# henryhungle/MTN

Measured on AMD Instinct MI355X. Metric: train-step samples/sec (d_model=512, 6L MTN), higher is better.
Workload: dtype bf16; 1 GPU; cfg2: d_model=512 N=6 h=8 d_ff=2048 |V|=3000 Q/H/C/T=20/128/40/20 frames=[32, 32] ft=[2048, 128]; batch_per_gpu=32, global_batch=32, parallelism=dp1, hip_graph=True, rccl_ranks=1

## Files before the change

mtn_amd/build.py:

```python
import os
import shutil
import subprocess
import sys
from concurrent.futures import ThreadPoolExecutor

HERE = os.path.dirname(os.path.abspath(__file__))
CSRC = os.path.join(HERE, "csrc")
OBJ = os.path.join(HERE, "build")
LIB = os.path.join(HERE, "libmtn_hip.so")
SOURCES = ["gemm.hip", "layernorm.hip", "attention.hip", "fused.hip", "fused_bwd.hip", "elementwise.hip", "sublayer.hip", "losshead.hip", "assemble.hip", "select.hip", "diverse.hip", "sample.hip", "score.hip", "constrain.hip", "ensemble.hip", "mbr.hip", "eval.hip", "scst.hip", "average.hip", "gradnorm.hip", "gradaccum.hip", "gemm_k512.hip", "decode.hip"]
FLAGS = ["--offload-arch=gfx950", "-O3", "-std=c++17", "-fPIC"]
SAFE_LIB = os.path.join(HERE, "libmtn_hip_safewaits.so")
SAFE_SOURCES = ["fused.hip", "fused_bwd.hip"]


def _headers_mtime() -> float:
    hs = [os.path.join(CSRC, f) for f in os.listdir(CSRC) if f.endswith(".h")] + [os.path.join(HERE, "..", "include", "mtn_hip.h")]
    return max(os.path.getmtime(h) for h in hs if os.path.exists(h))


def _stale() -> bool:
    if not os.path.exists(LIB):
        return True
    t = os.path.getmtime(LIB)
    deps = [os.path.join(CSRC, f) for f in os.listdir(CSRC)] + [os.path.join(HERE, "..", "include", "mtn_hip.h")]
    return any(os.path.getmtime(d) > t for d in deps if os.path.exists(d))


def build(force: bool = False, verbose: bool = True) -> str:
    if not force and not _stale():
        return LIB
    hipcc = shutil.which("hipcc") or "/opt/rocm/bin/hipcc"
    if not os.path.exists(hipcc):
        raise RuntimeError("hipcc not found: cannot build libmtn_hip.so")
    os.makedirs(OBJ, exist_ok=True)
    ht = _headers_mtime()
    todo = []
    for s in SOURCES:
        src, obj = os.path.join(CSRC, s), os.path.join(OBJ, s[:-4] + ".o")
        if force or not os.path.exists(obj) or os.path.getmtime(obj) < max(os.path.getmtime(src), ht):
            todo.append((src, obj))

    def cc(job):
        cmd = [hipcc] + FLAGS + ["-c", job[0], "-o", job[1]]
        if verbose:
            print(" ".join(cmd), flush=True)
        subprocess.check_call(cmd)

    with ThreadPoolExecutor(max(1, min(len(todo), os.cpu_count() or 1))) as ex:
        list(ex.map(cc, todo))
    cmd = [hipcc, "--offload-arch=gfx950", "-shared", "-fPIC", "-o", LIB + ".tmp"] + [os.path.join(OBJ, s[:-4] + ".o") for s in SOURCES]
    if verbose:
        print(" ".join(cmd), flush=True)
    subprocess.check_call(cmd)
    os.replace(LIB + ".tmp", LIB)
    return LIB


def build_safe_waits(verbose: bool = True) -> str:
    build(verbose=verbose)
    srcs = [os.path.join(CSRC, s) for s in SAFE_SOURCES]
    if os.path.exists(SAFE_LIB) and os.path.getmtime(SAFE_LIB) >= max(os.path.getmtime(LIB), max(os.path.getmtime(s) for s in srcs)):
        return SAFE_LIB
    hipcc = shutil.which("hipcc") or "/opt/rocm/bin/hipcc"

    def cc(s):
        obj = os.path.join(OBJ, s[:-4] + "_safewaits.o")
        cmd = [hipcc] + FLAGS + ["-DMTN_SAFE_WAITS", "-c", os.path.join(CSRC, s), "-o", obj]
        if verbose:
            print(" ".join(cmd), flush=True)
        subprocess.check_call(cmd)
        return obj

    with ThreadPoolExecutor(len(SAFE_SOURCES)) as ex:
        safe = list(ex.map(cc, SAFE_SOURCES))
    objs = safe + [os.path.join(OBJ, s[:-4] + ".o") for s in SOURCES if s not in SAFE_SOURCES]
    subprocess.check_call([hipcc, "--offload-arch=gfx950", "-shared", "-fPIC", "-o", SAFE_LIB + ".tmp"] + objs)
    os.replace(SAFE_LIB + ".tmp", SAFE_LIB)
    return SAFE_LIB


if __name__ == "__main__":
    build(force="--force" in sys.argv)
    print(LIB)
    print(build_safe_waits())
```

mtn_amd/csrc/common.h:

```cpp
#pragma once
#include <hip/hip_runtime.h>
#include <stdint.h>
#include <stdio.h>
#include <string.h>

#include "../../include/mtn_hip.h"

typedef unsigned short bf16_t;
typedef __attribute__((ext_vector_type(8))) __bf16 bf16x8_t;
typedef __attribute__((ext_vector_type(4))) float f32x4_t;

void mtn_set_error(const char* fmt, ...);
#define MTN_CHECK_ARG(cond, msg)                         \
    do {                                                 \
        if (!(cond)) {                                   \
            mtn_set_error("%s: %s", __func__, msg);      \
            return MTN_ERR_ARG;                          \
        }                                                \
    } while (0)
#define MTN_CHECK_LAUNCH()                                                        \
    do {                                                                          \
        hipError_t e__ = hipGetLastError();                                       \
        if (e__ != hipSuccess) {                                                  \
            mtn_set_error("%s: launch failed: %s", __func__, hipGetErrorString(e__)); \
            return MTN_ERR_LAUNCH;                                                \
        }                                                                         \
    } while (0)

struct MtnEnvVar { const char* name; int gen; bool set; char val[56]; };
const char* mtn_env_lookup(MtnEnvVar* v);
#define MTN_ENV(NAME) ([]() -> const char* { static MtnEnvVar v_ = {NAME, -1, false, {0}}; return mtn_env_lookup(&v_); }())

__device__ __forceinline__ float bf16_to_f32(bf16_t b) { return __uint_as_float(((uint32_t)b) << 16); }
__device__ __forceinline__ bf16_t f32_to_bf16(float f) {
    uint32_t u = __float_as_uint(f);
    if ((u & 0x7fffffffu) > 0x7f800000u) return (bf16_t)((u >> 16) | 0x40);
    u += 0x7fffu + ((u >> 16) & 1u);
    return (bf16_t)(u >> 16);
}

template <typename T> struct LP;
template <> struct LP<float> {
    static constexpr int EPV = 4;
    static constexpr int KSTEP = 16;
    __device__ static __forceinline__ float to_f32(float v) { return v; }
    __device__ static __forceinline__ float from_f32(float v) { return v; }
};
template <> struct LP<bf16_t> {
    static constexpr int EPV = 8;
    static constexpr int KSTEP = 32;
    __device__ static __forceinline__ float to_f32(bf16_t v) { return bf16_to_f32(v); }
    __device__ static __forceinline__ bf16_t from_f32(float v) { return f32_to_bf16(v); }
};

typedef __attribute__((ext_vector_type(4))) unsigned u32x4_t;
// ... 147 lines not shown
```

mtn_amd/csrc/fused.hip:

```cpp
#include "fused_common.h"
#include "gemm_k512_tile.h"

struct FhMember {
    int kind;
    int rows;
    int rows_per_wg;
    int nslice;
    int a, m, blk;
    int mt;
    int hg, sg;
    int late_v;
    int nks;
    int ncols;
    int ld_out;
    float eps;
    const float* x;
    const float* ln_a;
    const float* ln_b;
    const bf16_t* w;
    const float* bias;
    const bf16_t* mem;
    bf16_t* xn;
    float* mean;
    float* rstd;
    bf16_t* out;
    bf16_t* kv;
    const uint8_t* mask;
    long mask_sb, mask_sq;
    mtn_dropout drop;
    bf16_t* o;
    float* lse;
    int b_off;
};
struct FhGroup {
    int count;
    int stop;
#ifdef FH_TIMELINE
    unsigned long long* dbg;
#endif
    int wg_start[FH_MAX_MEMBERS + 1];
    FhMember m[FH_MAX_MEMBERS];
    int rider_base;
    GkRider kv;
};
static_assert(sizeof(FhGroup) <= 4096, "FhGroup travels by value in the kernel arguments");

struct FhLds { int gains, xn, xm, qi, ki, vi, mask, total; };
__host__ __device__ inline FhLds fh_lds_map(int mt, bool raw, int key_rows, int pad_rows, int mask_bytes, int ffn_blocks = 0, bool late_v = false) {
    FhLds L;
    L.gains = 0;
    L.xn = 4096 + 1024;
    const int krows = ((key_rows + pad_rows + 7) & ~7);
    if (late_v) {
        L.vi = L.xn;
        const int top = mt * 16 * FH_ROWB > krows * FH_HROWB ? mt * 16 * FH_ROWB : krows * FH_HROWB;
        L.xm = L.xn + top;
        L.qi = L.xm;
        L.ki = L.qi + mt * 16 * FH_HROWB;
        L.mask = L.ki + krows * FH_HROWB;
        L.total = L.mask + ((mask_bytes + 15) & ~15);
        return L;
    }
    L.xm = L.xn + mt * 16 * FH_ROWB;
    L.qi = L.xm + (raw ? mt * 16 * FH_ROWB : 0);
    L.ki = L.qi + mt * 16 * (ffn_blocks ? ffn_blocks * FH_HROWB : FH_HROWB);
    L.vi = L.ki + krows * FH_HROWB;
    L.mask = L.vi + krows * FH_HROWB;
    L.total = L.mask + ((mask_bytes + 15) & ~15);
// ... 474 lines not shown
        }
        __syncthreads();
        if (live && kr == 0) {
            for (int k = 1; k < nks; ++k) {
                const float* pk = (const float*)ki_s + (size_t)(pair * (nks - 1) + k - 1) * (FH_PART_FLOATS * 64) + lane;
                const float mo = pk[16 * 64], lo = pk[17 * 64];
                const float mn = fmaxf(mrun, mo);
                const float wa = (mrun == -INFINITY) ? 0.f : __expf(mrun - mn), wb = (mo == -INFINITY) ? 0.f : __expf(mo - mn);
                lrun = lrun * wa + lo * wb;
                mrun = mn;
#pragma unroll
                for (int nt = 0; nt < 4; ++nt)
#pragma unroll
                    for (int r = 0; r < 4; ++r) ot[nt][r] = ot[nt][r] * wa + pk[(nt * 4 + r) * 64] * wb;
            }
            finish(si, qt, ot, mrun, lrun);
        }
    }
    FH_STAMP(9);
    FH_STAMP_CLK(11);
}

template <int NP>
__global__ __launch_bounds__(FH_THREADS) void fused_head_fwd_kernel(const FhGroup G) {
    extern __shared__ __attribute__((aligned(16))) unsigned char smem[];
    FH_STAMP(0);
    FH_STAMP_CLK(10);
    if ((int)blockIdx.x >= G.wg_start[FH_MAX_MEMBERS]) {
        const int r = (int)blockIdx.x - G.rider_base;
        if (r >= 0 && r < G.kv.units) gk_rider_unit(G.kv, r, smem);
        return;
    }
    int g = 0;
    while (g + 1 < G.count && (int)blockIdx.x >= G.wg_start[g + 1]) ++g;
    const FhMember& M = G.m[g];
    const int t = (int)blockIdx.x - G.wg_start[g];
    const int xcd = t & 7, j = t >> 3;
    const int hpg = M.nslice / M.hg;
    const int slice = (xcd % M.hg) * hpg + (j % hpg), rb = (j / hpg) * M.sg + (xcd / M.hg);
    FH_STAMP(12);
    if (rb * M.rows_per_wg >= M.rows) return;
    if constexpr (NP == 4) {
        if (M.mt <= 2) fh_body<NP, 2>(G, M, slice, rb, smem);
        else fh_body<NP, 4>(G, M, slice, rb, smem);
    } else {
        if (M.mt <= 2) fh_body<NP, 2>(G, M, slice, rb, smem);
        else if (M.mt == 3) fh_body<NP, 3>(G, M, slice, rb, smem);
        else if (M.mt == 4) fh_body<NP, 4>(G, M, slice, rb, smem);
        else fh_body<NP, 5>(G, M, slice, rb, smem);
    }
}

static int fh_enabled = -1;
extern "C" int mtn_fused_enable(int on) {
    const int prev = fh_enabled;
    fh_enabled = on ? 1 : 0;
    return prev;
// ... 138 lines not shown
    }
    G.count = n;
    for (int i = n; i <= FH_MAX_MEMBERS; ++i) G.wg_start[i] = wgs;
    { static const int stop = [] { const char* e = getenv("MTN_FH_STOP"); return e ? atoi(e) : 0; }(); G.stop = stop; }
    P.wgs = wgs; P.np = np; P.lds = lds;
    return true;
}

int fh_group_eligible(int dtype, int n_mha, const mtn_mha_args* mha, int n_ffn, const mtn_ffn_args* ffn) {
    if (fh_env_off() || dtype != MTN_BF16) return 0;
    FhLaunch P;
    return fh_plan(n_mha, mha, n_ffn, ffn, P) ? 1 : 0;
}

template <int NP> static int fh_launch(const FhGroup& G, int wgs, size_t lds, hipStream_t s) {
    static bool attr = false;
    if (!attr) {
        if (hipFuncSetAttribute((const void*)fused_head_fwd_kernel<NP>, hipFuncAttributeMaxDynamicSharedMemorySize, FH_LDS_MAX) != hipSuccess) {
            mtn_set_error("fused_head_fwd_kernel: cannot raise the dynamic LDS limit");
            return MTN_ERR_LAUNCH;
        }
        attr = true;
    }
    hipLaunchKernelGGL((fused_head_fwd_kernel<NP>), dim3(wgs), dim3(FH_THREADS), lds, s, G);
    return MTN_OK;
}

static int fh_cu_count() {
    static int cus[64];
    int dev = 0;
    if (hipGetDevice(&dev) != hipSuccess || dev < 0 || dev >= 64) return 0;
    int n = __atomic_load_n(&cus[dev], __ATOMIC_RELAXED);
    if (n == 0) {
        if (hipDeviceGetAttribute(&n, hipDeviceAttributeMultiprocessorCount, dev) != hipSuccess || n < 1) n = -1;
        __atomic_store_n(&cus[dev], n, __ATOMIC_RELAXED);
    }
    return n > 0 ? n : 0;
}
static bool fh_rider_ffn_hosts() {
    const char* e = MTN_ENV("MTN_RIDER_FFN_HOSTS");
    return e ? e[0] != '0' : true;
}
static int fh_rider_slots(const FhLaunch& P) {
    if (!mtn_riders_enabled()) return 0;
    if (P.np == 4 && !fh_rider_ffn_hosts()) return 0;
    const int base = (P.wgs + 7) & ~7;
    int slots = fh_cu_count() - base;
// ... 25 lines not shown
```

mtn_amd/csrc/fused_bwd.hip:

```cpp
#include "fused_common.h"

#define FB_MAX_MEMBERS MTN_SUBLAYER_MAX_GROUP

struct FbMember {
    int rows, rows_per_wg;
    int a, m, blk, mt;
    int hg, sg;
    int self_attn;
    int ring;
    int ldq, ldkv;
    const bf16_t* dyl;
    const bf16_t* wot;
    const bf16_t* q;
    const bf16_t* k;
    const bf16_t* v;
    const bf16_t* o;
    const float* lse;
    const uint8_t* mask;
    long mask_sb, mask_sq;
    mtn_dropout drop;
    bf16_t* dq;
    bf16_t* dk;
    bf16_t* dv;
    const float* lnf;
    float* ln_part;
    int lnK;
};
// ... 486 lines not shown
                    }
                    if (lnon && 32 * qb + q2 * 16 < a) {
                        const int qc = q < a ? q : a - 1;
                        const float dqv[4] = {dqt[qb][q2][0] * scale, dqt[qb][q2][1] * scale, dqt[qb][q2][2] * scale, dqt[qb][q2][3] * scale};
                        float p1 = 0.f, p2 = 0.f;
                        ln_dot(dqv, qi_s, qrow0 + qc, 0, p1, p2);
                        ln_add(p1, p2, qrow0 + qc, q < a);
                    }
                }
        }
        if (rd == 0) FB_STAMP(11);
    }
    if (lnon) {
        __syncthreads();
        if (tid < R) {
            const float2* sl = (const float2*)rs_s + tid * 4;
            const float2 a0 = sl[0], a1 = sl[1], a2 = sl[2], a3 = sl[3];
            ((float2*)M.ln_part)[(size_t)(row0 + tid) * (FH_D / FH_DK) + slice] = make_float2((a0.x + a1.x) + (a2.x + a3.x), (a0.y + a1.y) + (a2.y + a3.y));
        }
    }
}

template <bool WIDE>
__global__ __launch_bounds__(FH_THREADS) void fused_head_bwd_kernel(const FbGroup G) {
    extern __shared__ __attribute__((aligned(16))) unsigned char smem[];
    int g = 0;
    while (g + 1 < G.count && (int)blockIdx.x >= G.wg_start[g + 1]) ++g;
    const FbMember& M = G.m[g];
    const int t = (int)blockIdx.x - G.wg_start[g];
    const int xcd = t & 7, j = t >> 3;
    const int hpg = (FH_D / FH_DK) / M.hg;
    const int slice = (xcd % M.hg) * hpg + (j % hpg), rb = (j / hpg) * M.sg + (xcd / M.hg);
    if (rb * M.rows_per_wg >= M.rows) return;
    if constexpr (WIDE) {
        if (M.ring) {
            if (M.a <= 32) fb_body<2, 1, true>(M, slice, rb, smem, G.stop, G.tl);
            else if (M.mt == 3) fb_body<3, 2, true>(M, slice, rb, smem, G.stop, G.tl);
            else if (M.mt == 4) fb_body<4, 2, true>(M, slice, rb, smem, G.stop, G.tl);
            else fb_body<5, 2, true>(M, slice, rb, smem, G.stop, G.tl);
            return;
        }
        if (M.a > 32) {
            if (M.mt == 3) fb_body<3, 2, false>(M, slice, rb, smem, G.stop, G.tl);
            else if (M.mt == 4) fb_body<4, 2, false>(M, slice, rb, smem, G.stop, G.tl);
            else fb_body<5, 2, false>(M, slice, rb, smem, G.stop, G.tl);
            return;
        }
    }
    if (M.mt <= 2) fb_body<2, 1, false>(M, slice, rb, smem, G.stop, G.tl);
    else if (M.mt == 3) fb_body<3, 1, false>(M, slice, rb, smem, G.stop, G.tl);
// ... 78 lines not shown
    P.wgs = wgs; P.lds = lds;
    return true;
}

int fb_group_eligible(int dtype, int n_mha, const mtn_mha_args* mha, const FbIo* io) {
    if (!fh_is_enabled() || dtype != MTN_BF16) return 0;
    FbLaunch P;
    return fb_plan(n_mha, mha, io, P) ? 1 : 0;
}

int fb_group_bwd_stage(int n_mha, const mtn_mha_args* mha, const FbIo* io, void* stream) {
    FbLaunch P;
    MTN_CHECK_ARG(fb_plan(n_mha, mha, io, P), "group outside the fused backward kernel's tiling");
    static bool attr = false;
    if (!attr) {
        if (hipFuncSetAttribute((const void*)fused_head_bwd_kernel<false>, hipFuncAttributeMaxDynamicSharedMemorySize, FB_LDS_MAX) != hipSuccess ||
            hipFuncSetAttribute((const void*)fused_head_bwd_kernel<true>, hipFuncAttributeMaxDynamicSharedMemorySize, FB_LDS_MAX) != hipSuccess) {
            mtn_set_error("fused_head_bwd_kernel: cannot raise the dynamic LDS limit");
            return MTN_ERR_LAUNCH;
        }
        attr = true;
    }
    FB_SELECT_LAUNCH(P);
    if (P.wide) hipLaunchKernelGGL(fused_head_bwd_kernel<true>, dim3(P.wgs), dim3(FH_THREADS), P.lds, (hipStream_t)stream, P.G);
    else hipLaunchKernelGGL(fused_head_bwd_kernel<false>, dim3(P.wgs), dim3(FH_THREADS), P.lds, (hipStream_t)stream, P.G);
    MTN_CHECK_LAUNCH();
    return MTN_OK;
}
```

mtn_amd/csrc/gemm.hip:

```cpp
#include <stdlib.h>
#include <type_traits>

#include "common.h"

struct GemmGroup {
    int count;
    int plain_tile_order;
    int epi_pre;
    unsigned char xcd_rg[MTN_GEMM_MAX_GROUP];
    int tile_start[MTN_GEMM_MAX_GROUP + 1];
    mtn_gemm_problem p[MTN_GEMM_MAX_GROUP];
};

int gemm_k512_try(int count, const mtn_gemm_problem* p, int min_tiles, hipStream_t s, int* tiles_out);

struct AdamSlot { float *p, *m, *v; void* lp; void* lpT; int ldT, write_grad; };
struct AdamGroup {
    const float* state;
    const float* grad_scale;
    float beta1, beta2, eps;
    int any;
    int lds_epilogue;
    AdamSlot a[MTN_GEMM_MAX_GROUP];
};
__device__ __forceinline__ AdamCoef adam_coef(const AdamGroup& G) { return adam_coef(G.state, G.grad_scale, G.beta1, G.beta2, G.eps); }
template <typename T>
__device__ __forceinline__ void adam4(const AdamSlot& A, const AdamCoef& c, bool vec, size_t o, int row, int col, int nv, const float (&g)[4]) {
    float pv[4], mv[4], vv[4];
    typedef __attribute__((ext_vector_type(4))) float nt4;
    if (vec) {
        const nt4 p_ = __builtin_nontemporal_load((const nt4*)(A.p + o)), m_ = __builtin_nontemporal_load((const nt4*)(A.m + o)),
                  v_ = __builtin_nontemporal_load((const nt4*)(A.v + o));
#pragma unroll
        for (int k = 0; k < 4; ++k) { pv[k] = p_[k]; mv[k] = m_[k]; vv[k] = v_[k]; }
    } else {
// ... 5 lines not shown
    if (vec) {
        __builtin_nontemporal_store(nt4{pv[0], pv[1], pv[2], pv[3]}, (nt4*)(A.p + o));
        __builtin_nontemporal_store(nt4{mv[0], mv[1], mv[2], mv[3]}, (nt4*)(A.m + o));
        __builtin_nontemporal_store(nt4{vv[0], vv[1], vv[2], vv[3]}, (nt4*)(A.v + o));
    } else {
        for (int k = 0; k < nv; ++k) { A.p[o + k] = pv[k]; A.m[o + k] = mv[k]; A.v[o + k] = vv[k]; }
    }
    if (A.lp) {
        T* op = (T*)A.lp + o;
        if (vec) {
            if constexpr (sizeof(T) == 2)
                *(uint2*)op = make_uint2((uint32_t)f32_to_bf16(pv[0]) | ((uint32_t)f32_to_bf16(pv[1]) << 16), (uint32_t)f32_to_bf16(pv[2]) | ((uint32_t)f32_to_bf16(pv[3]) << 16));
            else *(float4*)op = make_float4(pv[0], pv[1], pv[2], pv[3]);
        } else for (int k = 0; k < nv; ++k) op[k] = LP<T>::from_f32(pv[k]);
    }
    if (A.lpT) {
        T* tp = (T*)A.lpT + (size_t)col * A.ldT + row;
#pragma unroll
        for (int k = 0; k < 4; ++k)
            if (k < nv) tp[(size_t)k * A.ldT] = LP<T>::from_f32(pv[k]);
    }
}

__device__ __forceinline__ void xcd_tile(const GemmGroup& grp, int g, int t, int T, int tiles_m, int tiles_n, bool row_band, int& tm, int& tn) {
    int idx = t;
    if (!grp.plain_tile_order && T >= 16) {
        const int c = t & 7, r = t >> 3;
        const int per = T >> 3, rem = T & 7;
        idx = c * per + (c < rem ? c : rem) + r;
    }
    (void)g;
    if (row_band) { tm = idx / tiles_n; tn = idx - tm * tiles_n; }
    else { tn = idx / tiles_m; tm = idx - tn * tiles_m; }
}

__device__ __forceinline__ void xcd_tile2d(int rg, int t, int tiles_m, int tiles_n, int& tm, int& tn) {
    const int cg = 8 / rg;
    const int c = t & 7, r = t >> 3;
    const int bm = tiles_m / rg, bn = tiles_n / cg;
    const int ri = c / cg, ci = c - ri * cg;
    const int lm = r / bn, ln = r - lm * bn;
    tm = ri * bm + lm;
    tn = ci * bn + ln;
}
static int pick_xcd_rg(int first_tile, int tiles_m, int tiles_n, long M, long N) {
    if ((first_tile & 7) != 0 || ((tiles_m * tiles_n) & 7) != 0) return 0;
    int best = 0;
    double cost = 1e300;
    for (int rg = 1; rg <= 8; rg *= 2) {
        const int cg = 8 / rg;
        if (tiles_m % rg != 0 || tiles_n % cg != 0) continue;
        const double c = (double)cg * M + (double)rg * N;
        if (c < cost) { cost = c; best = rg; }
    }
    return best;
}
// ... 489 lines not shown
        const int gk = k0 + krow, gn = col0 + c * 8;
        unsigned voff = (gk < K && gn < N) ? (unsigned)gk * (unsigned)ld_bytes + (unsigned)gn * 2u : 0x80000000u;
        __builtin_amdgcn_raw_ptr_buffer_load_lds(rsrc, (lds_void_t*)(lds_tile + (j * NW + wave) * 1024), 16, voff, 0, 0, 0);
    }
}
template <int BN>
__device__ __forceinline__ uint4 kn_frag(const unsigned char* img, int n_off, int ks, int l15, int lg) {
    uint4 f;
#pragma unroll
    for (int r = 0; r < 2; ++r) {
        const int krow = ks * 32 + 8 * lg + 4 * r + (l15 >> 2);
        const int col = n_off + 4 * (l15 & 3);
        const int slot = (col >> 3) ^ kn_swz<BN>(krow);
        const unsigned addr = (unsigned)(size_t)(img + krow * (BN * 2) + slot * 16 + (col & 7) * 2);
        unsigned long long v;
        asm volatile("ds_read_b64_tr_b16 %0, %1" : "=v"(v) : "v"(addr));
        if (r == 0) { f.x = (unsigned)v; f.y = (unsigned)(v >> 32); }
        else { f.z = (unsigned)v; f.w = (unsigned)(v >> 32); }
    }
    return f;
}

template <typename T, int BM, int BN, int DMA_ROWB, bool BTR = false, int NBUF = 2, int NW = 4, bool LNE = false>
__global__ __launch_bounds__(64 * NW) void gemm_dma_kernel(const GemmGroup grp, const typename LnArg<LNE>::type lne) {
    constexpr int BK = DMA_ROWB / (int)sizeof(T);
    constexpr int WR = NW == 16 ? 4 : 2;
    constexpr int WC = NW / WR;
    constexpr int TM = BM / (16 * WR), TN = BN / (16 * WC);
    constexpr int A_BYTES = BM * DMA_ROWB, B_BYTES = BN * DMA_ROWB, STAGE_BYTES = A_BYTES + B_BYTES;
    constexpr int NDMA = (BM + BN) * DMA_ROWB / (1024 * NW);
    extern __shared__ __attribute__((aligned(16))) unsigned char smem[];
    const int tid = threadIdx.x;
    int g = 0;
    while (g + 1 < grp.count && (int)blockIdx.x >= grp.tile_start[g + 1]) ++g;
    const mtn_gemm_problem& P = grp.p[g];
    const int xcd_rg = grp.xcd_rg[g];
    const int first_tile = grp.tile_start[g];
    int lne_sl = 0;
    if constexpr (LNE) lne_sl = lne.slot_of[g];
    const int M = P.M, N = P.N, K = P.K;
    const int tiles_n = (N + BN - 1) / BN;
    const int t = (int)blockIdx.x - first_tile;
    const int tiles_m = (M + BM - 1) / BM;
    int tm_, tn_;
    if (xcd_rg) xcd_tile2d(xcd_rg, t, tiles_m, tiles_n, tm_, tn_);
    else xcd_tile(grp, g, t, tiles_m * tiles_n, tiles_m, tiles_n, M >= N, tm_, tn_);
    const int row0 = tm_ * BM, col0 = tn_ * BN;
    const int lane = tid & 63;
    const int wave = __builtin_amdgcn_readfirstlane(tid >> 6);
    const int wr = wave / WC, wc = wave % WC, lg = lane >> 4, l15 = lane & 15;
    const int lda_b = P.lda * (int)sizeof(T), ldb_b = P.ldb * (int)sizeof(T);
    const __amdgpu_buffer_rsrc_t rA = __builtin_amdgcn_make_buffer_rsrc((void*)P.A, 0, (M - 1) * lda_b + K * (int)sizeof(T), 0x00020000);
    const __amdgpu_buffer_rsrc_t rB = BTR ? __builtin_amdgcn_make_buffer_rsrc((void*)P.B, 0, (K - 1) * ldb_b + N * (int)sizeof(T), 0x00020000)
                                          : __builtin_amdgcn_make_buffer_rsrc((void*)P.B, 0, (N - 1) * ldb_b + K * (int)sizeof(T), 0x00020000);
    auto issue_b = [&](unsigned char* dst, int k0) {
        if constexpr (BTR) dma_issue_tile_kn<BN, DMA_ROWB, NW>(rB, dst, ldb_b, N, K, col0, k0, wave, lane);
        else dma_issue_tile<T, BN, DMA_ROWB, NW>(rB, dst, ldb_b, N, K, col0, k0, wave, lane);
    };

    f32x4_t acc[TM][TN];
#pragma unroll
    for (int i = 0; i < TM; ++i)
#pragma unroll
        for (int j = 0; j < TN; ++j) acc[i][j] = f32x4_t{0.f, 0.f, 0.f, 0.f};

    const int nstages = (K + BK - 1) / BK;
    auto issue_stage = [&](int st) {
        unsigned char* dst = smem + (st & (NBUF - 1)) * STAGE_BYTES;
        dma_issue_tile<T, BM, DMA_ROWB, NW>(rA, dst, lda_b, M, K, row0, st * BK, wave, lane);
        issue_b(dst + A_BYTES, st * BK);
    };
    for (int st = 0; st < (NBUF == 2 ? 2 : NBUF - 1) && st < nstages; ++st) issue_stage(st);
    typename std::conditional<LNE, LnConsumeLoads<TM, TN>, NoLn>::type lnq;
    float4 emit_u[TN], emit_c[TN];
    int lne_mode = 0;
    const bool vec_ok = ((N | P.ldc | (P.residual ? P.ldr : 0)) & 3) == 0;
    float4 pre_b[TN], pre_r[TM][TN];
    uint2 pre_g[TM][TN];
    bool pre_on = sizeof(T) == 2 && vec_ok && grp.epi_pre;
    if constexpr (LNE) {
        const int sl = lne_sl;
        if (sl != 0) {
            const LnEpiSlot& E = lne.s[sl - 1];
            lne_mode = E.mode;
            if (E.mode == MTN_LN_CONSUME) ln_consume_issue<TM, TN>(E, lnq, M, N, row0, row0 + wr * (BM / WR), col0 + wc * (BN / WC), l15, lg, tid, tid < 8 * BM);
            else {
#pragma unroll
                for (int j = 0; j < TN; ++j) {
                    const int col = col0 + wc * (BN / WC) + j * 16 + lg * 4;
                    const int cc = col < N ? col : 0;
                    emit_u[j] = *(const float4*)(E.fold + cc);
                    emit_c[j] = *(const float4*)(E.fold + N + cc);
                }
            }
        }
    }
    if (lne_mode == MTN_LN_CONSUME) pre_on = false;
#pragma unroll
    for (int j = 0; j < TN; ++j) {
        const int colj = col0 + wc * (BN / WC) + j * 16 + lg * 4, col = colj + 3 < N ? colj : 0;
        pre_b[j] = make_float4(0.f, 0.f, 0.f, 0.f);
        if (pre_on && P.bias) pre_b[j] = *(const float4*)(P.bias + col);
// ... 692 lines not shown
        }
    }
    const bool vec_ok = ((N | P.ldc | (P.residual ? P.ldr : 0)) & 3) == 0;
#pragma unroll
    for (int i = 0; i < 4; ++i) {
        const int row = row0 + wr * 64 + i * 16 + l15;
        if (row >= M) continue;
#pragma unroll
        for (int j = 0; j < 4; ++j) {
            const int col = col0 + wc * 64 + j * 16 + lg * 4;
            if (col >= N) continue;
            epilogue4<T>(P, ds, vec_ok && col + 3 < N, row, col, N, acc[i][j]);
        }
    }
}

static constexpr int G8_BK = 64;
static constexpr int G8_OP_BYTES = 128 * 128;
static constexpr int G8_STAGE = 2 * G8_OP_BYTES;
static constexpr int G8_NST = 4;
static constexpr int G8_LDS = G8_NST * G8_STAGE;

template <bool BTR, int NW = 16, bool LNE = false>
__global__ __launch_bounds__(64 * NW) void gemm_dma128x_kernel(const GemmGroup grp, const typename LnArg<LNE>::type lne) {
    constexpr int WR = NW / 4;
    constexpr int TM = 128 / (16 * WR);
    constexpr int IPW = 16 / NW;
    typedef bf16_t T;
    extern __shared__ __attribute__((aligned(16))) unsigned char smem[];
    const int tid = threadIdx.x;
    int g = 0;
    while (g + 1 < grp.count && (int)blockIdx.x >= grp.tile_start[g + 1]) ++g;
    const mtn_gemm_problem& P = grp.p[g];
    const int M = P.M, N = P.N, K = P.K;
    const int tiles_n = (N + 127) / 128, tiles_m = (M + 127) / 128;
    const int t = (int)blockIdx.x - grp.tile_start[g];
    int tm_, tn_;
    xcd_tile(grp, g, t, tiles_m * tiles_n, tiles_m, tiles_n, M >= N, tm_, tn_);
    const int row0 = tm_ * 128, col0 = tn_ * 128;
    const int lane = tid & 63;
    const int wave = __builtin_amdgcn_readfirstlane(tid >> 6);
    const int wr = wave >> 2, wc = wave & 3, lg = lane >> 4, l15 = lane & 15;
    const int lda_b = P.lda * 2, ldb_b = P.ldb * 2;
    const __amdgpu_buffer_rsrc_t rA = __builtin_amdgcn_make_buffer_rsrc((void*)P.A, 0, (M - 1) * lda_b + K * 2, 0x00020000);
    const __amdgpu_buffer_rsrc_t rB = BTR ? __builtin_amdgcn_make_buffer_rsrc((void*)P.B, 0, (K - 1) * ldb_b + N * 2, 0x00020000)
                                          : __builtin_amdgcn_make_buffer_rsrc((void*)P.B, 0, (N - 1) * ldb_b + K * 2, 0x00020000);
    auto issue_rows = [&](__amdgpu_buffer_rsrc_t rs, unsigned char* dst, int ld_bytes, int R, int r0, int k0) {
#pragma unroll
        for (int j = 0; j < IPW; ++j) {
            const int inst = j * NW + wave;
            const int row = inst * 8 + (lane >> 3);
            const int c = (lane & 7) ^ (row & 7);
            const int gk = k0 + c * 8;
            int grow = r0 + row;
            grow = grow < R ? grow : R - 1;
            unsigned voff = (gk < K) ? (unsigned)grow * (unsigned)ld_bytes + (unsigned)gk * 2u : 0x80000000u;
            __builtin_amdgcn_raw_ptr_buffer_load_lds(rs, (lds_void_t*)(dst + inst * 1024), 16, voff, 0, 0, 0);
        }
    };
    auto issue_kn = [&](unsigned char* dst, int k0) {
#pragma unroll
// ... 114 lines not shown
    bool has_aux; mtn_tt_aux aux; std::vector<mtn_tt_ln_unit> ln; std::vector<long> chunk_off; std::vector<int> chunk_len;
};
static std::vector<CensusEntry> g_census;
static std::vector<CensusTable> g_census_tables;
static bool g_census_on = false;
static int g_variant = 0, g_variant_tiles = 0;
enum { V_REG_NN = 0, V_REG_NT, V_REG_TN, V_REG_TT, V_DMA64, V_DMA3264, V_DMA32, V_TT_DMA, V_TT128, V_TT_DMA128, V_DMA128, V_DMA64H, V_DMA32H, V_TT_TABLE, V_K512, V_DMA128X, V_COUNT };
static const char* const g_variant_name[V_COUNT] = {
    "gemm_kernel<N,N> 64x64 reg-staged", "gemm_kernel<N,T>", "gemm_kernel<T,N>", "gemm_kernel<T,T> 64x64 reg-staged",
    "gemm_dma_kernel<64,64>", "gemm_dma_kernel<32,64>", "gemm_dma_kernel<32,32>", "gemm_tt_dma_kernel", "(gemm_tt128_kernel: removed in round 5)",
    "gemm_tt_dma128_kernel", "gemm_dma128_kernel", "gemm_dma_kernel<64,64> half stages", "gemm_dma_kernel<32,32> half stages", "gemm_tt_dma128_table_kernel", "gemm_k512_kernel", "gemm_dma128x_kernel (128x128, four stages)"};

template <typename T, int BM, int BN, int ROWB, bool BTR = false, int NBUF = 2, int NW = 4, bool LNE = false>
static int launch_dma_impl(const GemmGroup& grp, const typename LnArg<LNE>::type& lne, int tiles, hipStream_t s) {
    g_variant = (BM == 64) ? (ROWB == 512 ? V_DMA64 : V_DMA64H) : (BN == 64 ? V_DMA3264 : (ROWB == 512 ? V_DMA32 : V_DMA32H));
    g_variant_tiles = tiles;
    constexpr int LDS = NBUF * (BM + BN) * ROWB + (LNE ? LNE_LDS_EXTRA : 0);
    static bool attr_set = false;
    if (!attr_set && LDS > 64 * 1024) {
        hipError_t e = hipFuncSetAttribute((const void*)gemm_dma_kernel<T, BM, BN, ROWB, BTR, NBUF, NW, LNE>, hipFuncAttributeMaxDynamicSharedMemorySize, LDS);
        if (e != hipSuccess) { mtn_set_error("hipFuncSetAttribute: %s", hipGetErrorString(e)); return MTN_ERR_LAUNCH; }
        attr_set = true;
    }
    hipLaunchKernelGGL((gemm_dma_kernel<T, BM, BN, ROWB, BTR, NBUF, NW, LNE>), dim3(tiles), dim3(64 * NW), LDS, s, grp, lne);
    MTN_CHECK_LAUNCH();
    return MTN_OK;
}
template <typename T, int BM, int BN, int ROWB, bool BTR = false, int NBUF = 2, int NW = 4>
static int launch_dma(const GemmGroup& grp, int tiles, hipStream_t s, const LnEpiGroup* lne = nullptr) {
    if (lne) {
        if constexpr (sizeof(T) == 2 && NBUF == 2 && (64 * NW == 8 * BM || (NW == 16 && BM == 64)) && BM == BN)
            return launch_dma_impl<T, BM, BN, ROWB, BTR, NBUF, NW, true>(grp, *lne, tiles, s);
        mtn_set_error("mtn_gemm: no LayerNorm-epilogue form of this kernel (tile %d x %d, stage %d B, %d waves)", BM, BN, ROWB, NW);
        return MTN_ERR_ARG;
    }
    return launch_dma_impl<T, BM, BN, ROWB, BTR, NBUF, NW, false>(grp, NoLn{}, tiles, s);
}

template <typename T, int BM, int BN, int ROWB, int NBUF = 2, int NW = 4>
static int launch_dma_any(const GemmGroup& grp, int tiles, bool btr, hipStream_t s, const LnEpiGroup* lne = nullptr) {
    if constexpr (sizeof(T) == 2) {
        if (btr) return launch_dma<T, BM, BN, ROWB, true, NBUF, NW>(grp, tiles, s, lne);
    }
    return launch_dma<T, BM, BN, ROWB, false, NBUF, NW>(grp, tiles, s, lne);
}

static int retile(GemmGroup& grp, int bm, int bn, bool xcd2d = false) {
// ... 48 lines not shown
            int t128 = 0, kmax = 0;
            for (int i = 0; i < grp.count; ++i) {
                const mtn_gemm_problem& q = grp.p[i];
                ok = ok && !q.rowsum_out && q.K % 8 == 0 && q.K >= 256 && q.N % 8 == 0 && q.lda % 8 == 0 && q.ldb % 8 == 0 &&
                     (long)q.M * q.lda * 2 < (1L << 31) && (long)(bt ? q.K : q.N) * q.ldb * 2 < (1L << 31);
                t128 += ((q.M + 127) / 128) * ((q.N + 127) / 128);
                kmax = q.K > kmax ? q.K : kmax;
            }
            static int attr_state = 0;
            if (ok && t128 >= x_min && (xmin || kmax >= 768) && attr_state == 0) {
                const bool good =
                    hipFuncSetAttribute((const void*)gemm_dma128x_kernel<false, 16>, hipFuncAttributeMaxDynamicSharedMemorySize, G8_LDS) == hipSuccess &&
                    hipFuncSetAttribute((const void*)gemm_dma128x_kernel<true, 16>, hipFuncAttributeMaxDynamicSharedMemorySize, G8_LDS) == hipSuccess &&
                    hipFuncSetAttribute((const void*)gemm_dma128x_kernel<false, 8>, hipFuncAttributeMaxDynamicSharedMemorySize, G8_LDS) == hipSuccess &&
                    hipFuncSetAttribute((const void*)gemm_dma128x_kernel<true, 8>, hipFuncAttributeMaxDynamicSharedMemorySize, G8_LDS) == hipSuccess &&
                    hipFuncSetAttribute((const void*)gemm_dma128x_kernel<true, 16, true>, hipFuncAttributeMaxDynamicSharedMemorySize, G8_LDS + LNE_LDS_EXTRA) == hipSuccess;
                attr_state = good ? 1 : -1;
                if (!good) (void)hipGetLastError();
            }
            if (ok && t128 >= x_min && (xmin || kmax >= 768) && attr_state == 1) {
                GemmGroup g2 = grp;
                const int tiles = retile(g2, 128, 128);
                g_variant = V_DMA128X; g_variant_tiles = tiles;
                if (lne) hipLaunchKernelGGL((gemm_dma128x_kernel<true, 16, true>), dim3(tiles), dim3(1024), G8_LDS + LNE_LDS_EXTRA, s, g2, *lne);
                else {
                    if (bt) hipLaunchKernelGGL((gemm_dma128x_kernel<true, 16>), dim3(tiles), dim3(1024), G8_LDS, s, g2, NoLn{});
                    else hipLaunchKernelGGL((gemm_dma128x_kernel<false, 16>), dim3(tiles), dim3(1024), G8_LDS, s, g2, NoLn{});
                }
                MTN_CHECK_LAUNCH();
                return MTN_OK;
            }
        }
    }
    bool btr_ok = bt && sizeof(T) == 2;
    for (int i = 0; i < grp.count && btr_ok; ++i)
        btr_ok = grp.p[i].N % 8 == 0 && grp.p[i].ldb % 8 == 0 && (long)grp.p[i].K * grp.p[i].ldb * 2 < (1L << 31);
    if (lne && !(!at && dma_ok && (!bt || btr_ok))) {
        mtn_set_error("mtn_gemm: a LayerNorm epilogue needs the LDS-DMA kernel (bf16, a_trans = 0, aligned operands, a grid of at most 640 / 4096 tiles)");
        return MTN_ERR_ARG;
    }
    if (!at && dma_ok && (!bt || btr_ok)) {
        GemmGroup g2 = grp;
        const char* force = MTN_ENV("MTN_GEMM_TILE");
        int f = force ? atoi(force) : 0;
        if (lne_emit) f = 64;
        if (lne && f == 3264) f = 0;
        double b64 = 0, b32 = 0, wg32max = 0;
        int t64 = 0;
        for (int i = 0; i < grp.count; ++i) {
            const mtn_gemm_problem& q = grp.p[i];
// ... 537 lines not shown
```

Before: 9100 samples/s.

## Preload packed group-start header into SGPRs via kernarg preload for grouped kernels

Adds a 10-dword launch header to the grouped GEMM and fused head kernels. It packs the member count, flags and up to 18 block-start offsets as leading scalar arguments, and compiles those sources with the LLVM kernarg-preload option so the words arrive in SGPRs. The kernels find their group and read the tile-order and epilogue flags from these registers instead of scanning the by-value struct in kernarg memory, which cuts scalar loads at wave start. The member structs are also reordered and 64-byte aligned. This adds argument bytes, a fallback path, and a dependence on a compiler option, and the gain is limited to per-block startup latency.

New measurement: 9158 samples/s (median of 6 runs). About the same (+0.6%).

```diff
diff --git a/mtn_amd/build.py b/mtn_amd/build.py
--- a/mtn_amd/build.py
+++ b/mtn_amd/build.py
@@ -10,8 +10,16 @@
 LIB = os.path.join(HERE, "libmtn_hip.so")
 SOURCES = ["gemm.hip", "layernorm.hip", "attention.hip", "fused.hip", "fused_bwd.hip", "elementwise.hip", "sublayer.hip", "losshead.hip", "assemble.hip", "select.hip", "diverse.hip", "sample.hip", "score.hip", "constrain.hip", "ensemble.hip", "mbr.hip", "eval.hip", "scst.hip", "average.hip", "gradnorm.hip", "gradaccum.hip", "gemm_k512.hip", "decode.hip"]
 FLAGS = ["--offload-arch=gfx950", "-O3", "-std=c++17", "-fPIC"]
+PRELOAD_DWORDS = 10
+PRELOAD_SOURCES = ["gemm.hip", "fused.hip", "fused_bwd.hip"]
 SAFE_LIB = os.path.join(HERE, "libmtn_hip_safewaits.so")
 SAFE_SOURCES = ["fused.hip", "fused_bwd.hip"]
+
+
+def flags_for(source: str) -> list:
+    if source in PRELOAD_SOURCES:
+        return FLAGS + ["-mllvm", "-amdgpu-kernarg-preload-count=%d" % PRELOAD_DWORDS]
+    return list(FLAGS)
 
 
 def _headers_mtime() -> float:
@@ -39,10 +47,10 @@
     for s in SOURCES:
         src, obj = os.path.join(CSRC, s), os.path.join(OBJ, s[:-4] + ".o")
         if force or not os.path.exists(obj) or os.path.getmtime(obj) < max(os.path.getmtime(src), ht):
-            todo.append((src, obj))
+            todo.append((src, obj, s))
 
     def cc(job):
-        cmd = [hipcc] + FLAGS + ["-c", job[0], "-o", job[1]]
+        cmd = [hipcc] + flags_for(job[2]) + ["-c", job[0], "-o", job[1]]
         if verbose:
             print(" ".join(cmd), flush=True)
         subprocess.check_call(cmd)
@@ -66,7 +74,7 @@
 
     def cc(s):
         obj = os.path.join(OBJ, s[:-4] + "_safewaits.o")
-        cmd = [hipcc] + FLAGS + ["-DMTN_SAFE_WAITS", "-c", os.path.join(CSRC, s), "-o", obj]
+        cmd = [hipcc] + flags_for(s) + ["-DMTN_SAFE_WAITS", "-c", os.path.join(CSRC, s), "-o", obj]
         if verbose:
             print(" ".join(cmd), flush=True)
         subprocess.check_call(cmd)
@@ -80,6 +88,53 @@
     return SAFE_LIB
 
 
+def kernel_descriptors(path: str) -> dict:
+    import struct
+    blob = open(path, "rb").read()
+    magic = b"__CLANG_OFFLOAD_BUNDLE__"
+    out = {}
+    at = blob.find(magic)
+    while at >= 0:
+        n, = struct.unpack_from("<Q", blob, at + len(magic))
+        o = at + len(magic) + 8
+        for _ in range(n):
+            off, size, idlen = struct.unpack_from("<QQQ", blob, o)
+            o += 24
+            ident = blob[o:o + idlen].decode()
+            o += idlen
+            if "gfx950" in ident and size:
+                out.update(_elf_kernel_descriptors(blob[at + off:at + off + size]))
+        at = blob.find(magic, at + 1)
+    return out
+
+
+def _elf_kernel_descriptors(elf: bytes) -> dict:
+    import struct
+    assert elf[:4] == b"\x7fELF" and elf[4] == 2 and elf[5] == 1, "a little-endian ELF64 code object"
+    shoff, = struct.unpack_from("<Q", elf, 0x28)
+    shentsize, shnum, _ = struct.unpack_from("<HHH", elf, 0x3A)
+    secs = [struct.unpack_from("<IIQQQQIIQQ", elf, shoff + i * shentsize) for i in range(shnum)]
+    out = {}
+    for s in secs:
+        if s[1] != 2:
+            continue
+        strtab = secs[s[6]]
+        for i in range(s[5] // 24):
+            st_name, _info, _other, shndx, value, size = struct.unpack_from("<IBBHQQ", elf, s[4] + i * 24)
+            end = elf.index(b"\0", strtab[4] + st_name)
+            name = elf[strtab[4] + st_name:end].decode()
+            if not name.endswith(".kd") or size != 64 or shndx == 0 or shndx >= shnum:
+                continue
+            sec = secs[shndx]
+            kd = elf[sec[4] + value - sec[3]:sec[4] + value - sec[3] + 64]
+            lds, scratch = struct.unpack_from("<II", kd, 0)
+            rsrc1, = struct.unpack_from("<I", kd, 48)
+            preload, = struct.unpack_from("<H", kd, 58)
+            out[name[:-3]] = {"preload_length": preload & 0x7F, "preload_offset": preload >> 7, "vgprs": ((rsrc1 & 0x3F) + 1) * 8,
+                              "scratch": scratch, "lds": lds}
+    return out
+
+
 if __name__ == "__main__":
     build(force="--force" in sys.argv)
     print(LIB)
diff --git a/mtn_amd/csrc/common.h b/mtn_amd/csrc/common.h
--- a/mtn_amd/csrc/common.h
+++ b/mtn_amd/csrc/common.h
@@ -31,6 +31,42 @@
 const char* mtn_env_lookup(MtnEnvVar* v);
 #define MTN_ENV(NAME) ([]() -> const char* { static MtnEnvVar v_ = {NAME, -1, false, {0}}; return mtn_env_lookup(&v_); }())
 
+struct LaunchHead { unsigned w[10]; };
+#define MTN_HEAD_PARAMS unsigned hd0, unsigned hd1, unsigned hd2, unsigned hd3, unsigned hd4, unsigned hd5, unsigned hd6, unsigned hd7, unsigned hd8, unsigned hd9
+#define MTN_HEAD_ARGS(H) (H).w[0], (H).w[1], (H).w[2], (H).w[3], (H).w[4], (H).w[5], (H).w[6], (H).w[7], (H).w[8], (H).w[9]
+#define MTN_HEAD_PASS hd0, hd1, hd2, hd3, hd4, hd5, hd6, hd7, hd8, hd9
+static constexpr unsigned MTN_HEAD_VALID = 1u << 8;
+static constexpr int MTN_HEAD_FLAG_SHIFT = 9;
+static constexpr int MTN_HEAD_MAX_STARTS = 18;
+static inline LaunchHead mtn_launch_head(int count, const int* starts, int n, unsigned flags, int grid) {
+    LaunchHead H;
+    memset(&H, 0, sizeof(H));
+    const char* e = MTN_ENV("MTN_KERNARG_HEAD");
+    bool ok = !(e && e[0] == '0') && n <= MTN_HEAD_MAX_STARTS && count >= 1 && count <= 255 && grid <= 0xffff;
+    for (int i = 0; i < n && ok; ++i) ok = starts[i] >= 0 && starts[i] <= 0xffff;
+    H.w[0] = (unsigned)(count & 255) | (flags << MTN_HEAD_FLAG_SHIFT);
+    if (!ok) return H;
+    H.w[0] |= MTN_HEAD_VALID;
+    for (int i = 0; i < MTN_HEAD_MAX_STARTS; ++i) H.w[1 + i / 2] |= (unsigned)(i < n ? starts[i] : 0xffff) << (16 * (i & 1));
+    return H;
+}
+#define MTN_HEAD_START(i) ((((i) >> 1) == 0 ? hd1 : ((i) >> 1) == 1 ? hd2 : ((i) >> 1) == 2 ? hd3 : ((i) >> 1) == 3 ? hd4 : ((i) >> 1) == 4 ? hd5 : \
+                            ((i) >> 1) == 5 ? hd6 : ((i) >> 1) == 6 ? hd7 : ((i) >> 1) == 7 ? hd8 : hd9) >> (((i) & 1) * 16) & 0xffffu)
+template <int NMAX>
+__device__ __forceinline__ int mtn_head_find(unsigned bid, MTN_HEAD_PARAMS) {
+    static_assert(NMAX <= MTN_HEAD_MAX_STARTS, "the head holds 18 starts");
+    const int count = (int)(hd0 & 255u);
+    int g = 0;
+    if (count > 1) {
+#pragma unroll
+        for (int i = 1; i < NMAX; ++i) {
+            if ((i & 3) == 1 && i > 4) { if (count <= i) break; }
+            g += bid >= MTN_HEAD_START(i) ? 1 : 0;
+        }
+    }
+    return g;
+}
+
 __device__ __forceinline__ float bf16_to_f32(bf16_t b) { return __uint_as_float(((uint32_t)b) << 16); }
 __device__ __forceinline__ bf16_t f32_to_bf16(float f) {
     uint32_t u = __float_as_uint(f);
diff --git a/mtn_amd/csrc/fused.hip b/mtn_amd/csrc/fused.hip
--- a/mtn_amd/csrc/fused.hip
+++ b/mtn_amd/csrc/fused.hip
@@ -1,7 +1,7 @@
 #include "fused_common.h"
 #include "gemm_k512_tile.h"
 
-struct FhMember {
+struct alignas(64) FhMember {
     int kind;
     int rows;
     int rows_per_wg;
@@ -13,24 +13,24 @@
     int nks;
     int ncols;
     int ld_out;
+    int b_off;
     float eps;
     const float* x;
     const float* ln_a;
     const float* ln_b;
+    const float* bias;
+    const uint8_t* mask;
+    long mask_sb, mask_sq;
     const bf16_t* w;
-    const float* bias;
     const bf16_t* mem;
+    bf16_t* kv;
     bf16_t* xn;
     float* mean;
     float* rstd;
     bf16_t* out;
-    bf16_t* kv;
-    const uint8_t* mask;
-    long mask_sb, mask_sq;
     mtn_dropout drop;
     bf16_t* o;
     float* lse;
-    int b_off;
 };
 struct FhGroup {
     int count;
@@ -43,7 +43,7 @@
     int rider_base;
     GkRider kv;
 };
-static_assert(sizeof(FhGroup) <= 4096, "FhGroup travels by value in the kernel arguments");
+static_assert(sizeof(LaunchHead) + 64 + sizeof(FhGroup) <= 4096, "FhGroup travels by value in the kernel arguments, behind the launch head (and its alignment)");
 
 struct FhLds { int gains, xn, xm, qi, ki, vi, mask, total; };
 __host__ __device__ inline FhLds fh_lds_map(int mt, bool raw, int key_rows, int pad_rows, int mask_bytes, int ffn_blocks = 0, bool late_v = false) {
@@ -564,17 +564,20 @@
 }
 
 template <int NP>
-__global__ __launch_bounds__(FH_THREADS) void fused_head_fwd_kernel(const FhGroup G) {
+__global__ __launch_bounds__(FH_THREADS) void fused_head_fwd_kernel(MTN_HEAD_PARAMS, const FhGroup G) {
     extern __shared__ __attribute__((aligned(16))) unsigned char smem[];
     FH_STAMP(0);
     FH_STAMP_CLK(10);
-    if ((int)blockIdx.x >= G.wg_start[FH_MAX_MEMBERS]) {
-        const int r = (int)blockIdx.x - G.rider_base;
+    const bool head = (hd0 & MTN_HEAD_VALID) != 0;
+    const int members_end = head ? (int)MTN_HEAD_START(FH_MAX_MEMBERS) : G.wg_start[FH_MAX_MEMBERS];
+    if ((int)blockIdx.x >= members_end) {
+        const int r = (int)blockIdx.x - (head ? (int)MTN_HEAD_START(FH_MAX_MEMBERS + 1) : G.rider_base);
         if (r >= 0 && r < G.kv.units) gk_rider_unit(G.kv, r, smem);
         return;
     }
     int g = 0;
-    while (g + 1 < G.count && (int)blockIdx.x >= G.wg_start[g + 1]) ++g;
+    if (head) g = mtn_head_find<FH_MAX_MEMBERS>(blockIdx.x, MTN_HEAD_PASS);
+    else while (g + 1 < G.count && (int)blockIdx.x >= G.wg_start[g + 1]) ++g;
     const FhMember& M = G.m[g];
     const int t = (int)blockIdx.x - G.wg_start[g];
     const int xcd = t & 7, j = t >> 3;
@@ -759,7 +762,11 @@
         }
         attr = true;
     }
-    hipLaunchKernelGGL((fused_head_fwd_kernel<NP>), dim3(wgs), dim3(FH_THREADS), lds, s, G);
+    int starts[FH_MAX_MEMBERS + 2];
+    for (int i = 0; i <= FH_MAX_MEMBERS; ++i) starts[i] = G.wg_start[i];
+    starts[FH_MAX_MEMBERS + 1] = G.rider_base;
+    const LaunchHead H = mtn_launch_head(G.count, starts, FH_MAX_MEMBERS + 2, 0u, wgs);
+    hipLaunchKernelGGL((fused_head_fwd_kernel<NP>), dim3(wgs), dim3(FH_THREADS), lds, s, MTN_HEAD_ARGS(H), G);
     return MTN_OK;
 }
 
diff --git a/mtn_amd/csrc/fused_bwd.hip b/mtn_amd/csrc/fused_bwd.hip
--- a/mtn_amd/csrc/fused_bwd.hip
+++ b/mtn_amd/csrc/fused_bwd.hip
@@ -2,7 +2,7 @@
 
 #define FB_MAX_MEMBERS MTN_SUBLAYER_MAX_GROUP
 
-struct FbMember {
+struct alignas(64) FbMember {
     int rows, rows_per_wg;
     int a, m, blk, mt;
     int hg, sg;
@@ -535,10 +535,11 @@
 }
 
 template <bool WIDE>
-__global__ __launch_bounds__(FH_THREADS) void fused_head_bwd_kernel(const FbGroup G) {
+__global__ __launch_bounds__(FH_THREADS) void fused_head_bwd_kernel(MTN_HEAD_PARAMS, const FbGroup G) {
     extern __shared__ __attribute__((aligned(16))) unsigned char smem[];
     int g = 0;
-    while (g + 1 < G.count && (int)blockIdx.x >= G.wg_start[g + 1]) ++g;
+    if (hd0 & MTN_HEAD_VALID) g = mtn_head_find<FB_MAX_MEMBERS>(blockIdx.x, MTN_HEAD_PASS);
+    else while (g + 1 < G.count && (int)blockIdx.x >= G.wg_start[g + 1]) ++g;
     const FbMember& M = G.m[g];
     const int t = (int)blockIdx.x - G.wg_start[g];
     const int xcd = t & 7, j = t >> 3;
@@ -663,8 +664,9 @@
         attr = true;
     }
     FB_SELECT_LAUNCH(P);
-    if (P.wide) hipLaunchKernelGGL(fused_head_bwd_kernel<true>, dim3(P.wgs), dim3(FH_THREADS), P.lds, (hipStream_t)stream, P.G);
-    else hipLaunchKernelGGL(fused_head_bwd_kernel<false>, dim3(P.wgs), dim3(FH_THREADS), P.lds, (hipStream_t)stream, P.G);
+    const LaunchHead H = mtn_launch_head(P.G.count, P.G.wg_start, FB_MAX_MEMBERS + 1, 0u, P.wgs);
+    if (P.wide) hipLaunchKernelGGL(fused_head_bwd_kernel<true>, dim3(P.wgs), dim3(FH_THREADS), P.lds, (hipStream_t)stream, MTN_HEAD_ARGS(H), P.G);
+    else hipLaunchKernelGGL(fused_head_bwd_kernel<false>, dim3(P.wgs), dim3(FH_THREADS), P.lds, (hipStream_t)stream, MTN_HEAD_ARGS(H), P.G);
     MTN_CHECK_LAUNCH();
     return MTN_OK;
 }
diff --git a/mtn_amd/csrc/gemm.hip b/mtn_amd/csrc/gemm.hip
--- a/mtn_amd/csrc/gemm.hip
+++ b/mtn_amd/csrc/gemm.hip
@@ -11,6 +11,11 @@
     int tile_start[MTN_GEMM_MAX_GROUP + 1];
     mtn_gemm_problem p[MTN_GEMM_MAX_GROUP];
 };
+
+static constexpr unsigned GEMM_HEAD_EPI_PRE = 1u, GEMM_HEAD_PLAIN_TILES = 2u;
+static LaunchHead gemm_head(const GemmGroup& grp, int tiles) {
+    return mtn_launch_head(grp.count, grp.tile_start, MTN_GEMM_MAX_GROUP + 1, (grp.epi_pre ? GEMM_HEAD_EPI_PRE : 0u) | (grp.plain_tile_order ? GEMM_HEAD_PLAIN_TILES : 0u), tiles);
+}
 
 int gemm_k512_try(int count, const mtn_gemm_problem* p, int min_tiles, hipStream_t s, int* tiles_out);
 
@@ -62,16 +67,19 @@
     }
 }
 
-__device__ __forceinline__ void xcd_tile(const GemmGroup& grp, int g, int t, int T, int tiles_m, int tiles_n, bool row_band, int& tm, int& tn) {
+__device__ __forceinline__ void xcd_tile(bool plain_tile_order, int t, int T, int tiles_m, int tiles_n, bool row_band, int& tm, int& tn) {
     int idx = t;
-    if (!grp.plain_tile_order && T >= 16) {
+    if (!plain_tile_order && T >= 16) {
         const int c = t & 7, r = t >> 3;
         const int per = T >> 3, rem = T & 7;
         idx = c * per + (c < rem ? c : rem) + r;
     }
-    (void)g;
     if (row_band) { tm = idx / tiles_n; tn = idx - tm * tiles_n; }
     else { tn = idx / tiles_m; tm = idx - tn * tiles_m; }
+}
+__device__ __forceinline__ void xcd_tile(const GemmGroup& grp, int g, int t, int T, int tiles_m, int tiles_n, bool row_band, int& tm, int& tn) {
+    (void)g;
+    xcd_tile(grp.plain_tile_order != 0, t, T, tiles_m, tiles_n, row_band, tm, tn);
 }
 
 __device__ __forceinline__ void xcd_tile2d(int rg, int t, int tiles_m, int tiles_n, int& tm, int& tn) {
@@ -607,7 +615,7 @@
 }
 
 template <typename T, int BM, int BN, int DMA_ROWB, bool BTR = false, int NBUF = 2, int NW = 4, bool LNE = false>
-__global__ __launch_bounds__(64 * NW) void gemm_dma_kernel(const GemmGroup grp, const typename LnArg<LNE>::type lne) {
+__global__ __launch_bounds__(64 * NW) void gemm_dma_kernel(MTN_HEAD_PARAMS, const GemmGroup grp, const typename LnArg<LNE>::type lne) {
     constexpr int BK = DMA_ROWB / (int)sizeof(T);
     constexpr int WR = NW == 16 ? 4 : 2;
     constexpr int WC = NW / WR;
@@ -617,7 +625,9 @@
     extern __shared__ __attribute__((aligned(16))) unsigned char smem[];
     const int tid = threadIdx.x;
     int g = 0;
-    while (g + 1 < grp.count && (int)blockIdx.x >= grp.tile_start[g + 1]) ++g;
+    if (hd0 & MTN_HEAD_VALID) g = mtn_head_find<MTN_GEMM_MAX_GROUP>(blockIdx.x, MTN_HEAD_PASS);
+    else while (g + 1 < grp.count && (int)blockIdx.x >= grp.tile_start[g + 1]) ++g;
+    const bool head_epi_pre = (hd0 >> MTN_HEAD_FLAG_SHIFT) & GEMM_HEAD_EPI_PRE, head_plain = (hd0 >> MTN_HEAD_FLAG_SHIFT) & GEMM_HEAD_PLAIN_TILES;
     const mtn_gemm_problem& P = grp.p[g];
     const int xcd_rg = grp.xcd_rg[g];
     const int first_tile = grp.tile_start[g];
@@ -629,7 +639,7 @@
     const int tiles_m = (M + BM - 1) / BM;
     int tm_, tn_;
     if (xcd_rg) xcd_tile2d(xcd_rg, t, tiles_m, tiles_n, tm_, tn_);
-    else xcd_tile(grp, g, t, tiles_m * tiles_n, tiles_m, tiles_n, M >= N, tm_, tn_);
+    else xcd_tile(head_plain, t, tiles_m * tiles_n, tiles_m, tiles_n, M >= N, tm_, tn_);
     const int row0 = tm_ * BM, col0 = tn_ * BN;
     const int lane = tid & 63;
     const int wave = __builtin_amdgcn_readfirstlane(tid >> 6);
@@ -662,7 +672,7 @@
     const bool vec_ok = ((N | P.ldc | (P.residual ? P.ldr : 0)) & 3) == 0;
     float4 pre_b[TN], pre_r[TM][TN];
     uint2 pre_g[TM][TN];
-    bool pre_on = sizeof(T) == 2 && vec_ok && grp.epi_pre;
+    bool pre_on = sizeof(T) == 2 && vec_ok && head_epi_pre;
     if constexpr (LNE) {
         const int sl = lne_sl;
         if (sl != 0) {
@@ -1401,7 +1411,7 @@
 static constexpr int G8_LDS = G8_NST * G8_STAGE;
 
 template <bool BTR, int NW = 16, bool LNE = false>
-__global__ __launch_bounds__(64 * NW) void gemm_dma128x_kernel(const GemmGroup grp, const typename LnArg<LNE>::type lne) {
+__global__ __launch_bounds__(64 * NW) void gemm_dma128x_kernel(MTN_HEAD_PARAMS, const GemmGroup grp, const typename LnArg<LNE>::type lne) {
     constexpr int WR = NW / 4;
     constexpr int TM = 128 / (16 * WR);
     constexpr int IPW = 16 / NW;
@@ -1409,13 +1419,14 @@
     extern __shared__ __attribute__((aligned(16))) unsigned char smem[];
     const int tid = threadIdx.x;
     int g = 0;
-    while (g + 1 < grp.count && (int)blockIdx.x >= grp.tile_start[g + 1]) ++g;
+    if (hd0 & MTN_HEAD_VALID) g = mtn_head_find<MTN_GEMM_MAX_GROUP>(blockIdx.x, MTN_HEAD_PASS);
+    else while (g + 1 < grp.count && (int)blockIdx.x >= grp.tile_start[g + 1]) ++g;
     const mtn_gemm_problem& P = grp.p[g];
     const int M = P.M, N = P.N, K = P.K;
     const int tiles_n = (N + 127) / 128, tiles_m = (M + 127) / 128;
     const int t = (int)blockIdx.x - grp.tile_start[g];
     int tm_, tn_;
-    xcd_tile(grp, g, t, tiles_m * tiles_n, tiles_m, tiles_n, M >= N, tm_, tn_);
+    xcd_tile(((hd0 >> MTN_HEAD_FLAG_SHIFT) & GEMM_HEAD_PLAIN_TILES) != 0, t, tiles_m * tiles_n, tiles_m, tiles_n, M >= N, tm_, tn_);
     const int row0 = tm_ * 128, col0 = tn_ * 128;
     const int lane = tid & 63;
     const int wave = __builtin_amdgcn_readfirstlane(tid >> 6);
@@ -1576,7 +1587,8 @@
         if (e != hipSuccess) { mtn_set_error("hipFuncSetAttribute: %s", hipGetErrorString(e)); return MTN_ERR_LAUNCH; }
         attr_set = true;
     }
-    hipLaunchKernelGGL((gemm_dma_kernel<T, BM, BN, ROWB, BTR, NBUF, NW, LNE>), dim3(tiles), dim3(64 * NW), LDS, s, grp, lne);
+    const LaunchHead H = gemm_head(grp, tiles);
+    hipLaunchKernelGGL((gemm_dma_kernel<T, BM, BN, ROWB, BTR, NBUF, NW, LNE>), dim3(tiles), dim3(64 * NW), LDS, s, MTN_HEAD_ARGS(H), grp, lne);
     MTN_CHECK_LAUNCH();
     return MTN_OK;
 }
@@ -1671,10 +1683,11 @@
                 GemmGroup g2 = grp;
                 const int tiles = retile(g2, 128, 128);
                 g_variant = V_DMA128X; g_variant_tiles = tiles;
-                if (lne) hipLaunchKernelGGL((gemm_dma128x_kernel<true, 16, true>), dim3(tiles), dim3(1024), G8_LDS + LNE_LDS_EXTRA, s, g2, *lne);
+                const LaunchHead H = gemm_head(g2, tiles);
+                if (lne) hipLaunchKernelGGL((gemm_dma128x_kernel<true, 16, true>), dim3(tiles), dim3(1024), G8_LDS + LNE_LDS_EXTRA, s, MTN_HEAD_ARGS(H), g2, *lne);
                 else {
-                    if (bt) hipLaunchKernelGGL((gemm_dma128x_kernel<true, 16>), dim3(tiles), dim3(1024), G8_LDS, s, g2, NoLn{});
-                    else hipLaunchKernelGGL((gemm_dma128x_kernel<false, 16>), dim3(tiles), dim3(1024), G8_LDS, s, g2, NoLn{});
+                    if (bt) hipLaunchKernelGGL((gemm_dma128x_kernel<true, 16>), dim3(tiles), dim3(1024), G8_LDS, s, MTN_HEAD_ARGS(H), g2, NoLn{});
+                    else hipLaunchKernelGGL((gemm_dma128x_kernel<false, 16>), dim3(tiles), dim3(1024), G8_LDS, s, MTN_HEAD_ARGS(H), g2, NoLn{});
                 }
                 MTN_CHECK_LAUNCH();
                 return MTN_OK;
```
